# zubair-irshad/NeRF-MAE

Hardware: AMD Instinct MI355X
Metric: voxel-grids/sec (fwd+bwd+optimizer) swin_s 160^3 bf16 (higher is better)
Workload: dtype bf16; 1 GPU; swin_s MAE pretraining step, global batch 8 = 8 grid(s)/GPU of 4x160^3 RGB-sigma, mask_ratio 0.75, stochastic depth 0.1, AdamW+clip, DP=1 (BASELINE configs[2], the headline, read literally); global_batch=8, grids_per_gpu=8, resolution=160, parallelism=dp1, launch=hipgraph

## Files before the change

### nerf-mae_amd/csrc/common.hpp

```cpp
#pragma once
#include <hip/hip_runtime.h>
#include <stdint.h>

typedef unsigned short bf16_t;
typedef __attribute__((ext_vector_type(8))) short bf16x8;
typedef __attribute__((ext_vector_type(4))) short bf16x4;
typedef __attribute__((ext_vector_type(4))) float f32x4;
typedef __attribute__((ext_vector_type(4))) unsigned int u32x4;

#define NMH_DT_F32 0
#define NMH_DT_BF16 1

typedef float nmh_f2v __attribute__((ext_vector_type(2)));
typedef __bf16 nmh_b2v __attribute__((ext_vector_type(2)));
__device__ __forceinline__ unsigned pk_bf16(float lo, float hi) {
  nmh_f2v v = {lo, hi};
  return __builtin_bit_cast(unsigned, __builtin_convertvector(v, nmh_b2v));
}
__device__ __forceinline__ bf16_t f2bf(float f) { return __builtin_bit_cast(bf16_t, (__bf16)f); }
__device__ __forceinline__ float bf2f(bf16_t h) { return __uint_as_float(((unsigned)h) << 16); }

template <typename T> __device__ __forceinline__ float to_f(T v);
template <> __device__ __forceinline__ float to_f<float>(float v) { return v; }
template <> __device__ __forceinline__ float to_f<bf16_t>(bf16_t v) { return bf2f(v); }
// ... 71 lines not shown
  Frag<float> f;
  float4 a = *reinterpret_cast<const float4*>(lds + swz_off(row, 2 * g));
  float4 b = *reinterpret_cast<const float4*>(lds + swz_off(row, 2 * g + 1));
  f.v[0] = a.x; f.v[1] = a.y; f.v[2] = a.z; f.v[3] = a.w; f.v[4] = b.x; f.v[5] = b.y; f.v[6] = b.z; f.v[7] = b.w;
  return f;
}

typedef __attribute__((address_space(3))) bf16x4 lds_bf16x4;
__device__ __forceinline__ bf16x4 ds_read_tr16(const char* p) {
  return __builtin_amdgcn_ds_read_tr16_b64_v4i16((lds_bf16x4*)(__attribute__((address_space(3))) char*)p);
}
__device__ __forceinline__ Frag<bf16_t> lds_frag_t(const char* tile, int RS, int m0, int col0, int lane, bf16_t*) {
  const int g = lane >> 4, p = lane & 15;
  const char* a = tile + (m0 + 4 * g + (p >> 2)) * RS + (col0 + (p & 3) * 4) * 2;
  bf16x4 lo = ds_read_tr16(a);
  bf16x4 hi = ds_read_tr16(a + 16 * RS);
  Frag<bf16_t> f;
  f.v = __builtin_shufflevector(lo, hi, 0, 1, 2, 3, 4, 5, 6, 7);
  return f;
}
__device__ __forceinline__ Frag<float> lds_frag_t(const char* tile, int RS, int m0, int col0, int lane, float*) {
  const int g = lane >> 4, i = lane & 15;
  Frag<float> f;
#pragma unroll
  for (int j = 0; j < 8; ++j) {
    int m = m0 + 4 * g + (j & 3) + (j >> 2) * 16;
    f.v[j] = *reinterpret_cast<const float*>(tile + m * RS + (col0 + i) * 4);
  }
  return f;
}

struct TrFrag { bf16x4 lo, hi; };
__device__ __forceinline__ unsigned lds_addr_u(const void* p) { return (unsigned)(uintptr_t)(__attribute__((address_space(3))) const char*)p; }
template <int HI_OFF, int OFF0 = 0> __device__ __forceinline__ void tr_read_raw(TrFrag& f, unsigned addr) {
  static_assert(OFF0 >= 0 && OFF0 + HI_OFF < 65536, "ds offset field");
  asm volatile("ds_read_b64_tr_b16 %0, %1 offset:%2" : "=v"(f.lo) : "v"(addr), "n"(OFF0));
  asm volatile("ds_read_b64_tr_b16 %0, %1 offset:%2" : "=v"(f.hi) : "v"(addr), "n"(OFF0 + HI_OFF));
}
__device__ __forceinline__ float4 lds_read_f4_raw(const float* p) {
  float4 v;
  asm volatile("ds_read_b128 %0, %1\n\ts_waitcnt lgkmcnt(0)" : "=v"(v) : "v"(lds_addr_u(p)) : "memory");
  return v;
}
template <int OFF> __device__ __forceinline__ void tr_read1(bf16x4& d, unsigned addr) {
  static_assert(OFF >= 0 && OFF < 65536, "ds offset field");
  asm volatile("ds_read_b64_tr_b16 %0, %1 offset:%2" : "=v"(d) : "v"(addr), "n"(OFF));
}
__device__ __forceinline__ void tr_wait() { asm volatile("s_waitcnt lgkmcnt(0)" ::: "memory"); }
__device__ __forceinline__ void tr_pin(TrFrag& f) { asm volatile("" : "+v"(f.lo), "+v"(f.hi)); }
__device__ __forceinline__ Frag<bf16_t> tr_frag(const TrFrag& f) {
  Frag<bf16_t> r;
  r.v = __builtin_shufflevector(f.lo, f.hi, 0, 1, 2, 3, 4, 5, 6, 7);
  return r;
}

__device__ __forceinline__ float wave_sum(float v) {
#pragma unroll
  for (int o = 32; o > 0; o >>= 1) v += __shfl_xor(v, o, 64);
  return v;
}
__device__ __forceinline__ float gelu_f(float x) { return 0.5f * x * (1.0f + erff(x * 0.70710678118654752f)); }
__device__ __forceinline__ float gelu_grad_f(float x) {
  return 0.5f * (1.0f + erff(x * 0.70710678118654752f)) + x * 0.39894228040143268f * __expf(-0.5f * x * x);
}
__device__ __forceinline__ void erf_as_parts(float z, float& erfz, float& e) {
  const float az = fabsf(z);
  const float t = __builtin_amdgcn_rcpf(1.0f + 0.3275911f * az);
  e = __expf(-az * az);
  float p = 1.061405429f;
  p = p * t - 1.453152027f; p = p * t + 1.421413741f; p = p * t - 0.284496736f; p = p * t + 0.254829592f;
  erfz = copysignf(1.0f - p * t * e, z);
}
__device__ __forceinline__ float gelu_fast_f(float x) {
  float er, e;
  erf_as_parts(x * 0.70710678118654752f, er, e);
  return 0.5f * x * (1.0f + er);
}
__device__ __forceinline__ float gelu_grad_fast_f(float x) {
  float er, e;
  erf_as_parts(x * 0.70710678118654752f, er, e);
  return 0.5f * (1.0f + er) + x * 0.39894228040143268f * e;
}

struct NmhPerDeviceOnce {
  bool done[64] = {};
  static int dev() { int d = 0; if (hipGetDevice(&d) != hipSuccess || d < 0 || d >= 64) d = 0; return d; }
  bool need() const { return !done[dev()]; }
  void set() { done[dev()] = true; }
};
#ifdef __HIPCC__
static __global__ void nmh_zero_kernel(unsigned* p, long n) {
  for (long i = (long)blockIdx.x * blockDim.x + threadIdx.x; i < n; i += (long)gridDim.x * blockDim.x) p[i] = 0u;
}
extern char* g_nmh_arena_base;
extern size_t g_nmh_arena_bytes;
static inline hipError_t nmh_zero_async(void* p, size_t bytes, hipStream_t st) {
  const long n = (long)(bytes / 4);
  if (n <= 0) return hipSuccess;
  if (g_nmh_arena_bytes && (char*)p >= g_nmh_arena_base && (char*)p + bytes <= g_nmh_arena_base + g_nmh_arena_bytes) return hipSuccess;
  long nb = (n + 255) / 256;
  if (nb > 2048) nb = 2048;
  hipLaunchKernelGGL(nmh_zero_kernel, dim3((unsigned)nb), dim3(256), 0, st, (unsigned*)p, n);
  return hipGetLastError();
}
#endif
#define NMH_CHECK_LAUNCH() do { hipError_t e_ = hipGetLastError(); if (e_ != hipSuccess) return (int)e_; } while (0)
// ... 1 lines not shown
```

### nerf-mae_amd/csrc/conv48.hip

```cpp
#include "common.hpp"
#include "kernels.hpp"
#include <cstdlib>
#include <type_traits>

__device__ __forceinline__ unsigned c48_fdiv(unsigned n, const FDiv& f) { return f.sh < 0 ? n : (__umulhi(n, f.M) >> f.sh); }

namespace c48 {
constexpr int TZ = 4, TY = 8, TX = 16, HY = TY + 2, HX = TX + 2;
constexpr int LINE = HX * 96 + 16, PLANE = HY * LINE + 16, HALO = (TZ + 2) * PLANE;
constexpr int NSTEP = 41, CSTEPS = 9, WCHUNK = CSTEPS * 3 * 1024;
constexpr int LDS_BYTES = HALO + 2 * WCHUNK + 2 * 96 * 4;
constexpr int NLINE = (TZ + 2) * HY;
constexpr int LPW = (NLINE + 7) / 8;
constexpr int HREG = 2 * LPW;
static_assert(HREG == 16 && HX * 6 > 64 && HX * 6 <= 128, "the halo request schedule (4 per weight chunk 0-3) assumes 16 loads per thread, two per line");
static_assert(LINE % 32 == 16 && PLANE % 32 == 16, "bank-half alternation");
static_assert(LDS_BYTES <= 163840, "LDS budget");
}

struct C48Args {
  const bf16_t* X; const bf16_t* Wk; bf16_t* Y;
  int B, D, H, W, tz, ty, tx;
  long total;
  FDiv dtx, dty, dtz;
  int accumulate;
  double* stats_acc;
  const bf16_t* Y1; const float* stats1; float slope;
  float inv_slope;
  long wk_sample_stride;
  int ncib, ncob, ldx, ldy;
  int cosplit;
};

__device__ __forceinline__ void c48_tile_origin(const C48Args& a, long t, int& b, int& z0, int& y0, int& x0) {
  const unsigned tu = (unsigned)t;
  const unsigned r1 = c48_fdiv(tu, a.dtx), xt = tu - r1 * (unsigned)a.tx;
  const unsigned r2 = c48_fdiv(r1, a.dty), yt = r1 - r2 * (unsigned)a.ty;
  const unsigned r3 = c48_fdiv(r2, a.dtz), zt = r2 - r3 * (unsigned)a.tz;
  b = __builtin_amdgcn_readfirstlane((int)r3);
  z0 = __builtin_amdgcn_readfirstlane((int)zt * c48::TZ);
  y0 = __builtin_amdgcn_readfirstlane((int)yt * c48::TY);
  x0 = __builtin_amdgcn_readfirstlane((int)xt * c48::TX);
}

template <int, bool MB = false, bool RB = false, bool CZ = false>
__global__ __launch_bounds__(512) void conv48_kernel(C48Args a) {
  using namespace c48;
  constexpr long WBLK = (long)NSTEP * 3 * 512;
  extern __shared__ __attribute__((aligned(16))) char smem[];
  char* halo = smem;
  char* wbuf = smem + HALO;
  const int tid = threadIdx.x, lane = tid & 63, wave = tid >> 6, g = lane >> 4, li = lane & 15;

  const int nx = 8, xcd = blockIdx.x % nx, jb = blockIdx.x / nx, jstride = gridDim.x / nx;
  const bool split = MB && a.cosplit;
  const long total = split ? a.total * a.ncob : a.total;
  const long per = (total + nx - 1) / nx;
  const long tbeg = (long)xcd * per, tend = (tbeg + per < total) ? tbeg + per : total;

  uint4 hreg[HREG];
  const unsigned vox_bytes = MB ? (unsigned)a.ldx * 2u : 96u;
  const unsigned sample_bytes = (unsigned)a.D * a.H * a.W * vox_bytes;
  constexpr unsigned OOB = 0x80000000u;
  const int wv = __builtin_amdgcn_readfirstlane(wave);
  unsigned hv0 = OOB, hv1 = OOB;
  auto halo_voff = [&](int x0, int cib) {
    int lv = lane;
    asm volatile("" : "+v"(lv));
    const int c1 = lv + 64;
    const int hxa = (lv * 43) >> 8, hxb = (c1 * 43) >> 8;
    const int xa = x0 - 1 + hxa, xb = x0 - 1 + hxb;
    const unsigned cofs = MB ? (unsigned)cib * 96u : 0u;
    hv0 = (unsigned)xa < (unsigned)a.W ? (unsigned)xa * vox_bytes + (unsigned)(lv - hxa * 6) * 16u + cofs : OOB;
    hv1 = (c1 < HX * 6 && (unsigned)xb < (unsigned)a.W) ? (unsigned)xb * vox_bytes + (unsigned)(c1 - hxb * 6) * 16u + cofs : OOB;
  };
  auto halo_gload_one = [&](int i, int b, int z0, int y0, unsigned bytes) {
    const int j = i >> 1, l = wv + 8 * j;
    const int hz = (l * 205) >> 11, hy = l - hz * HY;
    const int z = z0 - 1 + hz, y = y0 - 1 + hy;
    const unsigned lok = (unsigned)(l < NLINE) & (unsigned)((unsigned)z < (unsigned)a.D) & (unsigned)((unsigned)y < (unsigned)a.H);
    const unsigned lmask = 0u - lok;
    const __amdgpu_buffer_rsrc_t rs = __builtin_amdgcn_make_buffer_rsrc((void*)(a.X + (long)b * (sample_bytes / 2)), 0, (int)(bytes & lmask), 0x00020000);
    const unsigned soff = ((unsigned)((z * a.H + y) * a.W) * vox_bytes) & lmask;
    hreg[i] = __builtin_bit_cast(uint4, __builtin_amdgcn_raw_buffer_load_b128(rs, (int)((i & 1) ? hv1 : hv0), (int)soff, 0));
  };
  auto halo_sstore = [&]() {
#pragma unroll
    for (int j = 0; j < LPW; ++j) {
      const int l = wv + 8 * j;
      if (l < NLINE) {
        const int hz = (l * 205) >> 11, hy = l - hz * HY;
        char* const p = halo + hz * PLANE + hy * LINE + lane * 16;
        *reinterpret_cast<uint4*>(p) = hreg[2 * j];
        if (lane < HX * 6 - 64) *reinterpret_cast<uint4*>(p + 1024) = hreg[2 * j + 1];
      }
    }
  };
  auto w_dma = [&](const bf16_t* wblk, int ck, int buf) {
    const int nunits = ((ck < 4) ? CSTEPS : (NSTEP - 4 * CSTEPS)) * 192;
    const char* src = reinterpret_cast<const char*>(wblk) + (long)ck * CSTEPS * 3072;
    char* dst = wbuf + buf * WCHUNK;
    for (int u0 = wave * 64; u0 < nunits; u0 += 512) {
      __builtin_amdgcn_global_load_lds((const __attribute__((address_space(1))) void*)(src + (long)(u0 + lane) * 16),
                                       (__attribute__((address_space(3))) void*)(dst + u0 * 16), 16, 0, 0);
    }
  };

  auto w_dma_one = [&](const bf16_t* wblk, int ck, int buf, int j) {
    const int nunits = ((ck < 4) ? CSTEPS : (NSTEP - 4 * CSTEPS)) * 192;
    const int u0 = wave * 64 + 512 * j;
    int lv = lane;
    asm volatile("" : "+v"(lv));
    if (u0 < nunits)
      __builtin_amdgcn_global_load_lds((const __attribute__((address_space(1))) void*)(reinterpret_cast<const char*>(wblk) + (long)ck * CSTEPS * 3072 + (long)(u0 + lv) * 16),
                                       (__attribute__((address_space(3))) void*)(wbuf + buf * WCHUNK + u0 * 16), 16, 0, 0);
  };

  for (int i = tid; i < HALO / 16; i += 512) reinterpret_cast<uint4*>(halo)[i] = make_uint4(0, 0, 0, 0);
  if (tid < 192) reinterpret_cast<float*>(smem + HALO + 2 * WCHUNK)[tid] = 0.f;
  __syncthreads();

  long t = tbeg + jb;
  if (t >= tend) return;
  int cb, cz0, cy0, cx0;
  c48_tile_origin(a, split ? t / a.ncob : t, cb, cz0, cy0, cx0);
  int cob = split ? (int)(t % a.ncob) : 0, cib = 0;
  const bf16_t* const wfirst = MB ? a.Wk + (long)cob * a.ncib * ((long)NSTEP * 3 * 512) : a.Wk + (long)cb * a.wk_sample_stride;
  halo_voff(cx0, 0);
#pragma unroll
  for (int i = 0; i < HREG; ++i) halo_gload_one(i, cb, cz0, cy0, sample_bytes);
  w_dma(wfirst, 0, 0);
  halo_sstore();
  __syncthreads();
  int wb = 0;

  const int z_l = wave >> 1, y_l = (wave & 1) * 4;
  const int base0 = z_l * PLANE + y_l * LINE + li * 96;
  int rowoff[2];
#pragma unroll
  for (int q = 0; q < 2; ++q) { const int r = 4 * q + g; rowoff[q] = (r / 3) * PLANE + (r % 3) * LINE; }
  const int row8 = 2 * PLANE + 2 * LINE;

  float* const sacc = reinterpret_cast<float*>(smem + HALO + 2 * WCHUNK);
  int st_b = -1, scur = 0;
  auto stats_flush = [&]() {
    if (st_b >= 0 && tid < 96) {
      float v = sacc[scur * 96 + tid];
      const float sacc_even = (RB && CZ) ? __shfl(v, (tid & 63) & ~1, 64) : 0.f;
      sacc[scur * 96 + tid] = 0.f;
      if (RB && (tid & 1)) {
        if constexpr (CZ) v -= a.stats1[(long)st_b * 96 + tid - 1] * sacc_even;
        v *= a.stats1[(long)st_b * 96 + tid];
      }
      atomicAdd(a.stats_acc + (long)st_b * 96 + tid, (double)v);
    }
  };
  auto row_sum = [](float v) -> float {
    v += __builtin_bit_cast(float, __builtin_amdgcn_update_dpp(0, __builtin_bit_cast(int, v), 0x111, 0xf, 0xf, true));
    v += __builtin_bit_cast(float, __builtin_amdgcn_update_dpp(0, __builtin_bit_cast(int, v), 0x112, 0xf, 0xf, true));
    v += __builtin_bit_cast(float, __builtin_amdgcn_update_dpp(0, __builtin_bit_cast(int, v), 0x114, 0xf, 0xf, true));
    v += __builtin_bit_cast(float, __builtin_amdgcn_update_dpp(0, __builtin_bit_cast(int, v), 0x118, 0xf, 0xf, true));
    return v;
  };
  f32x4 acc[4][3];
  for (;;) {
    long tn = t + jstride;
    int nco = 0, nci = 0;
    if (MB) {
      nci = cib + 1; nco = cob; tn = t;
      if (nci == a.ncib) { nci = 0; ++nco; }
      if (split) {
        if (nci == 0) { tn = t + jstride; nco = (int)(tn % a.ncob); }
      } else if (nco == a.ncob) { nco = 0; tn = t + jstride; }
    }
    const bool has_next = tn < tend;
    int nb = cb, nz0 = cz0, ny0 = cy0, nx0 = cx0;
    if (has_next && (!MB || tn != t)) c48_tile_origin(a, split ? tn / a.ncob : tn, nb, nz0, ny0, nx0);
    const unsigned nbytes = has_next ? sample_bytes : 0u;
    halo_voff(nx0, nci);
    const bf16_t* const wcur = MB ? a.Wk + (long)(cob * a.ncib + cib) * WBLK : a.Wk + (long)cb * a.wk_sample_stride;
    const bf16_t* const wnxt = MB ? a.Wk + (long)(nco * a.ncib + nci) * WBLK : a.Wk + (long)nb * a.wk_sample_stride;
    if (!MB || cib == 0) {
#pragma unroll
      for (int i = 0; i < 4; ++i)
#pragma unroll
        for (int n = 0; n < 3; ++n) acc[i][n] = f32x4{0.f, 0.f, 0.f, 0.f};
    }

    auto a_off = [&](int s) -> int {
      if (s < 36) {
        const int q = s / 18, c = s % 18;
        return base0 + rowoff[q] + (c / 6) * 96 + (c % 6) * 16;
      }
      int c = 4 * (s - 36) + g;
      c = c > 17 ? 17 : c;
      const int c6 = (c * 43) >> 8;
      return base0 + row8 + c6 * 96 + (c - 6 * c6) * 16;
    };
    Frag<bf16_t> bf[2][3], af[2][4];
    auto ld_frags = [&](int buf, const char* wsrc, int sl, int s) {
      const int ao = a_off(s);
#pragma unroll
      for (int n = 0; n < 3; ++n) bf[buf][n].v = *reinterpret_cast<const bf16x8*>(wsrc + (sl * 3 + n) * 1024 + lane * 16);
#pragma unroll
      for (int i = 0; i < 4; ++i) af[buf][i].v = *reinterpret_cast<const bf16x8*>(halo + ao + i * LINE);
    };
#pragma unroll
    for (int ck = 0; ck < 5; ++ck) {
      const int nxt = (ck < 4) ? ck + 1 : 0;
      const char* wsrc = wbuf + ((wb + ck) & 1) * WCHUNK;
      constexpr int NST4 = NSTEP - 4 * CSTEPS;
      const int nst = (ck < 4) ? CSTEPS : NST4;
      const int hbase = 4 * ck;
      const int hcnt = ck < 4 ? 4 : 0;
      ld_frags(0, wsrc, 0, ck * CSTEPS);
#pragma unroll
      for (int sl = 0; sl < CSTEPS; ++sl) {
        if (sl < nst) {
          if (sl + 1 < nst) ld_frags((sl + 1) & 1, wsrc, sl + 1, ck * CSTEPS + sl + 1);
          if (sl < 4) w_dma_one(ck < 4 ? wcur : wnxt, nxt, (wb + ck + 1) & 1, sl);
          if (sl >= 4) {
            const int k = (hcnt == 4) ? (sl == 4 ? 0 : sl == 5 ? 1 : sl == 6 ? 2 : sl == 8 ? 3 : -1) : (hcnt == 3) ? (sl == 4 ? 0 : sl == 6 ? 1 : sl == 8 ? 2 : -1) : -1;
            if (k >= 0) halo_gload_one(hbase + k, nb, nz0, ny0, nbytes);
          }
#pragma unroll
          for (int i = 0; i < 4; ++i)
#pragma unroll
            for (int n = 0; n < 3; ++n) mma(acc[i][n], bf[sl & 1][n], af[sl & 1][i]);
        }
      }
      if (hcnt == 4) asm volatile("s_waitcnt vmcnt(4)" ::: "memory");
      else if (hcnt == 3) asm volatile("s_waitcnt vmcnt(3)" ::: "memory");
      else asm volatile("s_waitcnt vmcnt(0)" ::: "memory");
      __builtin_amdgcn_s_barrier();
    }
    wb ^= 1;

    if (has_next) halo_sstore();

    if (!MB || cib == a.ncib - 1) {
      const int b = cb, z0 = cz0, y0 = cy0, x0 = cx0;
      const int z = z0 + z_l, x = x0 + li;
      const bool stats = !MB && a.stats_acc;
      if (stats && b != st_b) {
        stats_flush();
        if (st_b >= 0) scur ^= 1;
        st_b = b;
      }
      const int ldy = MB ? a.ldy : 48;
      bf16_t* const dst0 = a.Y + ((((long)b * a.D + z) * a.H + (y0 + y_l)) * a.W + x) * ldy + (MB ? cob * 48 : 0) + 12 * g;
      const long rowstride = (long)a.W * ldy;
      const bool zx_ok = z < a.D && x < a.W;
      auto epilogue = [&](auto with_stats) {
        constexpr bool ST = decltype(with_stats)::value;
        uint4 yA[RB ? 4 : 1]; uint2 yB[RB ? 4 : 1]; float4 mu4[RB ? 3 : 1];
        unsigned wk[RB ? 4 : 1][6];
        if constexpr (RB) {
          const bf16_t* const y1p = a.Y1 + (dst0 - a.Y);
#pragma unroll
          for (int i = 0; i < 4; ++i)
            if (zx_ok && y0 + y_l + i < a.H) {
              yA[i] = *reinterpret_cast<const uint4*>(y1p + i * rowstride);
              yB[i] = *reinterpret_cast<const uint2*>(y1p + i * rowstride + 8);
            }
          const float4* sp = reinterpret_cast<const float4*>(a.stats1 + ((long)b * 48 + 12 * g) * 2);
#pragma unroll
          for (int q = 0; q < 3; ++q) {
            const float4 p0 = sp[2 * q], p1 = sp[2 * q + 1];
            mu4[q] = make_float4(p0.x, p0.z, p1.x, p1.z);
          }
        }
        float st1[ST ? 3 : 1][4], st2[ST ? 3 : 1][4];
        if (ST) {
#pragma unroll
          for (int n = 0; n < 3; ++n)
#pragma unroll
            for (int r = 0; r < 4; ++r) { st1[ST ? n : 0][r] = 0.f; st2[ST ? n : 0][r] = 0.f; }
        }
#pragma unroll
        for (int i = 0; i < 4; ++i) {
          if (zx_ok && y0 + y_l + i < a.H) {
            bf16_t* dst = dst0 + i * rowstride;
            float v[3][4];
#pragma unroll
            for (int n = 0; n < 3; ++n)
#pragma unroll
              for (int r = 0; r < 4; ++r) v[n][r] = acc[i][n][r];
            if (a.accumulate) {
              const uint4 o = *reinterpret_cast<const uint4*>(dst);
              const uint2 o2 = *reinterpret_cast<const uint2*>(dst + 8);
              const unsigned ow[6] = {o.x, o.y, o.z, o.w, o2.x, o2.y};
// ... 9 lines not shown
#pragma unroll
              for (int q = 0; q < 6; ++q) wk[i][q] = w6[q];
            }
            if (ST && !RB) {
#pragma unroll
              for (int q = 0; q < 6; ++q) {
                const float q0 = __uint_as_float(w6[q] << 16), q1 = __uint_as_float(w6[q] & 0xffff0000u);
                st1[ST ? q >> 1 : 0][(q & 1) * 2] += q0; st1[ST ? q >> 1 : 0][(q & 1) * 2 + 1] += q1;
                st2[ST ? q >> 1 : 0][(q & 1) * 2] += q0 * q0; st2[ST ? q >> 1 : 0][(q & 1) * 2 + 1] += q1 * q1;
              }
            }
          }
        }
        if constexpr (RB) {
#pragma unroll
          for (int i = 0; i < 4; ++i)
            if (zx_ok && y0 + y_l + i < a.H) {
              const unsigned yw[6] = {yA[i].x, yA[i].y, yA[i].z, yA[i].w, yB[i].x, yB[i].y};
#pragma unroll
              for (int q = 0; q < 6; ++q) {
                const float d0 = __uint_as_float(wk[i][q] << 16), d1 = __uint_as_float(wk[i][q] & 0xffff0000u);
                const float m0 = (q & 1) ? mu4[q >> 1].z : mu4[q >> 1].x, m1 = (q & 1) ? mu4[q >> 1].w : mu4[q >> 1].y;
                const float y0v = __uint_as_float(yw[q] << 16), y1v = __uint_as_float(yw[q] & 0xffff0000u);
                if constexpr (CZ) {
                  const float g0 = d0 * (y0v > 0.f ? 1.0f : a.slope), g1 = d1 * (y1v > 0.f ? 1.0f : a.slope);
                  st1[q >> 1][(q & 1) * 2] += g0; st1[q >> 1][(q & 1) * 2 + 1] += g1;
                  st2[q >> 1][(q & 1) * 2] += d0 * y0v; st2[q >> 1][(q & 1) * 2 + 1] += d1 * y1v;
                } else {
                const float t0 = y0v - m0, t1 = y1v - m1;
                const float g0 = d0 * (t0 > 0.f ? 1.0f : a.slope), g1 = d1 * (t1 > 0.f ? 1.0f : a.slope);
                st1[q >> 1][(q & 1) * 2] += g0; st1[q >> 1][(q & 1) * 2 + 1] += g1;
                st2[q >> 1][(q & 1) * 2] += g0 * t0; st2[q >> 1][(q & 1) * 2 + 1] += g1 * t1;
                }
              }
            }
        }
        if (ST) {
#pragma unroll
          for (int n = 0; n < 3; ++n)
#pragma unroll
            for (int r = 0; r < 4; ++r) {
              const float a1 = row_sum(st1[ST ? n : 0][r]), a2 = row_sum(st2[ST ? n : 0][r]);
              if (li == 15) {
                float* dst = sacc + scur * 96 + (12 * g + 4 * n + r) * 2;
                atomicAdd(dst, a1);
                atomicAdd(dst + 1, a2);
              }
            }
        }
      };
      if (stats || RB) epilogue(std::true_type{});
      else epilogue(std::false_type{});
    }
    cb = nb; cz0 = nz0; cy0 = ny0; cx0 = nx0;
    __syncthreads();
    if (!has_next) break;
    t = tn; cob = nco; cib = nci;
  }
  if (a.stats_acc) stats_flush();
}


int k_conv48(const void* X, const void* Wk, void* Y, int B, int D, int H, int W, int accumulate, double* stats_acc, hipStream_t st,
             const void* Y1, const float* stats1, float slope, long wk_sample_stride, int centered) {
  using namespace c48;
  C48Args a;
  a.Y1 = (const bf16_t*)Y1; a.stats1 = stats1; a.slope = slope;
  a.inv_slope = slope != 0.f ? 1.0f / slope : 0.f; a.wk_sample_stride = wk_sample_stride;
  if (Y1 && (!stats1 || !stats_acc || accumulate)) return -1;
  if ((centered && !Y1) || (wk_sample_stride && (Y1 || accumulate))) return -1;
  a.X = (const bf16_t*)X; a.Wk = (const bf16_t*)Wk; a.Y = (bf16_t*)Y;
  a.B = B; a.D = D; a.H = H; a.W = W;
  a.tz = (D + TZ - 1) / TZ; a.ty = (H + TY - 1) / TY; a.tx = (W + TX - 1) / TX;
  a.total = (long)B * a.tz * a.ty * a.tx;
  if (a.total >= (1L << 31) || (long)D * H * W * 96 >= (1L << 31)) return -2;
  a.dtx = make_fdiv((unsigned)a.tx); a.dty = make_fdiv((unsigned)a.ty); a.dtz = make_fdiv((unsigned)a.tz);
  a.accumulate = accumulate;
  a.stats_acc = stats_acc;
  a.ncib = a.ncob = 1; a.ldx = a.ldy = 48; a.cosplit = 0;
  if (stats_acc) {
    hipError_t e = nmh_zero_async(stats_acc, sizeof(double) * 2 * 48 * B, st);
    if (e != hipSuccess) return (int)e;
  }
  static NmhPerDeviceOnce attr_set;
  if (attr_set.need()) {
    hipError_t e = hipFuncSetAttribute((const void*)conv48_kernel<0>, hipFuncAttributeMaxDynamicSharedMemorySize, LDS_BYTES);
    if (e != hipSuccess) return (int)e;
    attr_set.set();
  }
  long nb = a.total < 256 ? ((a.total + 7) / 8 * 8) : 256;
  if (Y1) {
    static NmhPerDeviceOnce attr_rb;
    if (attr_rb.need()) {
      hipError_t e = hipFuncSetAttribute((const void*)conv48_kernel<0, false, true>, hipFuncAttributeMaxDynamicSharedMemorySize, LDS_BYTES);
      if (e != hipSuccess) return (int)e;
      attr_rb.set();
    }
    if (centered) {
      static NmhPerDeviceOnce attr_cz;
      if (attr_cz.need()) {
        hipError_t e = hipFuncSetAttribute((const void*)conv48_kernel<0, false, true, true>, hipFuncAttributeMaxDynamicSharedMemorySize, LDS_BYTES);
        if (e != hipSuccess) return (int)e;
        attr_cz.set();
      }
      hipLaunchKernelGGL((conv48_kernel<0, false, true, true>), dim3((unsigned)nb), dim3(512), LDS_BYTES, st, a);
    } else hipLaunchKernelGGL((conv48_kernel<0, false, true>), dim3((unsigned)nb), dim3(512), LDS_BYTES, st, a);
    NMH_CHECK_LAUNCH();
    return 0;
  }
  hipLaunchKernelGGL(conv48_kernel<0>, dim3((unsigned)nb), dim3(512), LDS_BYTES, st, a);
  NMH_CHECK_LAUNCH();
  return 0;
// ... 258 lines not shown
    for (; bb < nblocks; ++bb) t8[bb & 7] += src[(long)bb * w48::PARTIAL];
    s = ((t8[0] * sc[0] + t8[1] * sc[1]) + (t8[2] * sc[2] + t8[3] * sc[3])) + ((t8[4] * sc[4] + t8[5] * sc[5]) + (t8[6] * sc[6] + t8[7] * sc[7]));
  }
  dW[((long)(os * 48 + ct * 16 + row) * Cin + cs * 48 + cit * 16 + col) * 27 + tap] += s;
}

long k_conv48_wgrad_ws_floats() { return 256L * w48::PARTIAL; }

static int launch_wgrad_halo(const void* dY, const void* X, float* dW, float* ws, int B, int D, int H, int W, int Cin, int Cout, hipStream_t st, const float* scale_stats = nullptr) {
  using namespace w48;
  W48Args a;
  a.X = (const bf16_t*)X; a.dY = (const bf16_t*)dY; a.ws = ws;
  a.B = B; a.D = D; a.H = H; a.W = W;
  a.tz = (D + TZ - 1) / TZ; a.ty = (H + TY - 1) / TY; a.tx = (W + TX - 1) / TX;
  a.total = (long)B * a.tz * a.ty * a.tx;
  if (a.total >= (1L << 31)) return -2;
  a.dtx = make_fdiv((unsigned)a.tx); a.dty = make_fdiv((unsigned)a.ty); a.dtz = make_fdiv((unsigned)a.tz);
  a.ldx = Cin; a.ldy = Cout; a.nci = Cin / 48;
  const int nsub = (Cin / 48) * (Cout / 48);
  static NmhPerDeviceOnce attr_set;
  if (attr_set.need()) {
    hipError_t e = hipFuncSetAttribute((const void*)conv48_wgrad_kernel, hipFuncAttributeMaxDynamicSharedMemorySize, LDS_BYTES);
    if (e != hipSuccess) return (int)e;
    attr_set.set();
  }
  if (scale_stats) {
    const long tps = (long)a.tz * a.ty * a.tx;
    if (nsub != 1 || B < 1 || 8 % B || tps % (8 / B)) return -2;
  }
  int nb;
  if (nsub == 1) nb = a.total < 256 ? (int)((a.total + 7) / 8 * 8) : 256;
  else {
    static const int side_wgs = [] { const char* e = getenv("NMH_W48_SIDE_WGS"); const int v = e ? atoi(e) : 128; return v < 1 ? 1 : (v > 256 ? 256 : v); }();
    nb = side_wgs / nsub;
    if (nb < 1) nb = 1;
    if (nb > a.total) nb = (int)a.total;
  }
  hipLaunchKernelGGL(conv48_wgrad_kernel, dim3(nb, nsub), dim3(512), LDS_BYTES, st, a);
  NMH_CHECK_LAUNCH();
  hipLaunchKernelGGL(conv48_wgrad_reduce_kernel, dim3((PARTIAL + 255) / 256, nsub), dim3(256), 0, st, ws, dW, nb, a.nci, Cin, scale_stats, B);
  NMH_CHECK_LAUNCH();
  return 0;
}
int k_conv48_wgrad(const void* dY, const void* X, float* dW, float* ws, int B, int D, int H, int W, hipStream_t st, const float* scale_stats) {
  return launch_wgrad_halo(dY, X, dW, ws, B, D, H, W, 48, 48, st, scale_stats);
}

__global__ void conv48_pack_scaled_kernel(const float* __restrict__ W, const float* __restrict__ stats, bf16_t* __restrict__ out) {
  constexpr int IMG = c48::NSTEP * 3 * 512;
  const int b = blockIdx.y;
  for (int iw = blockIdx.x * 256 + threadIdx.x; iw < IMG; iw += gridDim.x * 256) {
    const int j = iw & 7, lane = (iw >> 3) & 63, sn = iw >> 9;
    const int nt = sn % 3, st = sn / 3, g = lane >> 4, li = lane & 15, n = 12 * (li >> 2) + 4 * nt + (li & 3);
    int r, c;
    if (st < 36) { r = 4 * (st / 18) + g; c = st % 18; } else { r = 8; c = 4 * (st - 36) + g; }
    float v = 0.f;
    if (c < 18) {
      const int tap = r * 3 + c / 6, k = (c % 6) * 8 + j;
      v = W[((long)n * 48 + k) * 27 + tap] * stats[((long)b * 48 + k) * 2 + 1];
    }
    out[(long)b * IMG + iw] = f2bf(v);
  }
}
int k_conv48_pack_scaled(const float* W, const float* stats, void* out, int B, hipStream_t st) {
  hipLaunchKernelGGL(conv48_pack_scaled_kernel, dim3(62, B), dim3(256), 0, st, W, stats, (bf16_t*)out);
  NMH_CHECK_LAUNCH();
  return 0;
}
int k_conv3_wgrad_halo(const void* dY, const void* X, float* dW, float* ws, int B, int D, int H, int W, int Cin, int Cout, hipStream_t st) {
  if (Cin % 48 || Cout % 48 || (Cin / 48) * (Cout / 48) > 256 || (double)D * H * W * Cin * 2 >= 4294967296.0) return -2;
  return launch_wgrad_halo(dY, X, dW, ws, B, D, H, W, Cin, Cout, st);
}
```

### nerf-mae_amd/csrc/misc.hip

```cpp
#include "common.hpp"
#include "kernels.hpp"

static inline unsigned ew_blocks(long total, int cap = 16384) { long nb = (total + 255) / 256; return (unsigned)(nb > cap ? cap : (nb < 1 ? 1 : nb)); }

template <typename T> __global__ __launch_bounds__(256) void embed_gather_kernel(const float* __restrict__ x, T* __restrict__ A, int B, int R) {
  extern __shared__ __attribute__((aligned(16))) char esm[];
  const int g = R >> 2;
  constexpr int ROWB = 256 * (int)sizeof(T) + 8;
  const int line = blockIdx.x;
  const int ty = line % g, tz = (line / g) % g, b = line / (g * g);
  for (int idx = threadIdx.x; idx < 64 * g; idx += 256) {
    const int q = idx / g, tx = idx - q * g;
    const int ci = q >> 4, kz = (q >> 2) & 3, ky = q & 3;
    const float4 v = *reinterpret_cast<const float4*>(x + ((((long)b * 4 + ci) * R + 4 * tz + kz) * R + 4 * ty + ky) * (long)R + 4 * tx);
    T* o = reinterpret_cast<T*>(esm + tx * ROWB) + q * 4;
    o[0] = from_f<T>(v.x); o[1] = from_f<T>(v.y); o[2] = from_f<T>(v.z); o[3] = from_f<T>(v.w);
  }
  __syncthreads();
  constexpr int V8 = 256 * (int)sizeof(T) / 8;
  unsigned long long* out = reinterpret_cast<unsigned long long*>(A + (long)line * g * 256);
  for (int idx = threadIdx.x; idx < g * V8; idx += 256) {
    const int tx = idx / V8, c = idx - tx * V8;
    out[idx] = *reinterpret_cast<const unsigned long long*>(esm + tx * ROWB + c * 8);
  }
// ... 456 lines not shown
  p.g = tokmask ? g : 0;
  hipLaunchKernelGGL(step_params_kernel, dim3(n ? (n + 255) / 256 : 1), dim3(256), 0, st, p, tokmask, hyper_dev, ext_dev);
  NMH_CHECK_LAUNCH();
  return 0;
}

__global__ void grad_f32_to_bf16_kernel(const float* __restrict__ src, bf16_t* __restrict__ dst, long n8) {
  for (long i = (long)blockIdx.x * blockDim.x + threadIdx.x; i < n8; i += (long)gridDim.x * blockDim.x) {
    float v[8];
    Vec8<float>::load(src + i * 8, v);
    Vec8<bf16_t>::store(dst + i * 8, v);
  }
}
__global__ void grad_bf16_to_f32_kernel(const bf16_t* __restrict__ src, float* __restrict__ dst, long n8, float scale) {
  for (long i = (long)blockIdx.x * blockDim.x + threadIdx.x; i < n8; i += (long)gridDim.x * blockDim.x) {
    float v[8];
    Vec8<bf16_t>::load(src + i * 8, v);
#pragma unroll
    for (int j = 0; j < 8; ++j) v[j] *= scale;
    Vec8<float>::store(dst + i * 8, v);
  }
}
int k_grad_cast(int to_bf16, const void* src, void* dst, long n, float scale, hipStream_t st) {
  if (n % 8 || ((uintptr_t)src | (uintptr_t)dst) & 15) return -2;
  if (to_bf16) hipLaunchKernelGGL(grad_f32_to_bf16_kernel, dim3(ew_blocks(n / 8)), dim3(256), 0, st, (const float*)src, (bf16_t*)dst, n / 8);
  else hipLaunchKernelGGL(grad_bf16_to_f32_kernel, dim3(ew_blocks(n / 8)), dim3(256), 0, st, (const bf16_t*)src, (float*)dst, n / 8, scale);
  NMH_CHECK_LAUNCH();
  return 0;
}
__global__ void fill_kernel(float* p, float v, long n) {
  for (long i = (long)blockIdx.x * blockDim.x + threadIdx.x; i < n; i += (long)gridDim.x * blockDim.x) p[i] = v;
}
int k_fill_f32(float* p, float v, long n, hipStream_t st) {
  hipLaunchKernelGGL(fill_kernel, dim3(ew_blocks(n)), dim3(256), 0, st, p, v, n);
  NMH_CHECK_LAUNCH();
  return 0;
}

__device__ __forceinline__ long pack_src_index(const PackDesc& d, long il) {
  const unsigned i = (unsigned)il, d0 = (unsigned)d.d0, d1 = (unsigned)d.d1, d2 = (unsigned)d.d2;
  switch (d.mode) {
    case 1: { unsigned c = i / d0, r = i - c * d0; return (long)(r * d1 + c); }
    case 2: { unsigned t2 = i / d1, ci = i - t2 * d1, co = t2 / 27u, t = t2 - co * 27u; return (long)((co * d1 + ci) * 27u + t); }
    case 3: { unsigned t2 = i / d0, co = i - t2 * d0, ci = t2 / 27u, t = t2 - ci * 27u; return (long)((co * d1 + ci) * 27u + (26u - t)); }
    case 4: { unsigned t2 = i / d0, ci = i - t2 * d0, t = t2 / d1, co = t2 - t * d1; return (long)((ci * d1 + co) * d2 + t); }
    case 5: { unsigned n = d1 * d2, ci = i / n, r = i - ci * n, t = r / d1, co = r - t * d1; return (long)((ci * d1 + co) * d2 + t); }
    case 6: case 7: {
      constexpr unsigned IMG = 41u * 3u * 512u;
      const unsigned blk = i / IMG, iw = i - blk * IMG;
      const unsigned nkb = (d.mode == 6 ? d1 : d0) / 48u, ob = blk / nkb, kb = blk - ob * nkb;
      const int j = (int)(iw & 7), lane = (int)((iw >> 3) & 63);
      const unsigned sn = iw >> 9;
      const int nt = (int)(sn % 3), st = (int)(sn / 3), g = lane >> 4, li = lane & 15, n = (int)ob * 48 + 12 * (li >> 2) + 4 * nt + (li & 3);
      int r, c;
      if (st < 36) { r = 4 * (st / 18) + g; c = st % 18; } else { r = 8; c = 4 * (st - 36) + g; }
      if (c >= 18) return -1;
      const int tap = r * 3 + c / 6, k = (int)kb * 48 + (c % 6) * 8 + j;
      return d.mode == 6 ? ((long)n * d1 + k) * 27 + tap : ((long)k * d1 + n) * 27 + (26 - tap);
    }
    case 10: { unsigned r = i / d1; return r < d0 ? (long)i : -1; }
    case 11: { unsigned c = i / d2, r = i - c * d2; return r < d0 ? (long)(r * d1 + c) : -1; }
    case 12: { unsigned ci = i & 7u, t2 = i >> 3, co = t2 / d2, t = t2 - co * d2; return ci < d1 ? (long)((co * d1 + ci) * d2 + t) : -1; }
    case 8: case 9: {
      const int j = (int)(i & 7), lane = (int)((i >> 3) & 63);
      const unsigned sn = i >> 9;
      const int nt = (int)(sn & 3), sg = (int)(sn >> 2), blk = sg / 54, st = sg - blk * 54;
      const int ncs = (d.mode == 8 ? (int)d1 : (int)d0) / 64, os = blk / ncs, cs = blk - os * ncs;
      const int g = lane >> 4, li = lane & 15, n = os * 64 + 16 * (li >> 2) + 4 * nt + (li & 3), k = cs * 64 + (st & 1) * 32 + 8 * g + j, tap = st >> 1;
      return d.mode == 8 ? ((long)n * d1 + k) * 27 + tap : ((long)k * d1 + n) * 27 + (26 - tap);
    }
    default: return il;
  }
}
template <typename T> __global__ void pack_kernel(const PackDesc* descs, const int* blk2desc, const long* blkstart) {
  const PackDesc d = descs[blk2desc[blockIdx.x]];
  const long base = blkstart[blockIdx.x];
  T* dst = (T*)d.dst;
  if (d.mode == 1) {
    __shared__ float tile[32][33];
    const int tcn = (d.d1 + 31) >> 5, tr = (int)(base / tcn), tc = (int)(base - (long)tr * tcn);
    const int r0 = tr * 32, c0 = tc * 32, tx = threadIdx.x & 31, ty = threadIdx.x >> 5;
#pragma unroll
    for (int r = ty; r < 32; r += 8)
      if (r0 + r < d.d0 && c0 + tx < d.d1) tile[r][tx] = d.src[(long)(r0 + r) * d.d1 + c0 + tx];
    __syncthreads();
#pragma unroll
    for (int c = ty; c < 32; c += 8)
      if (c0 + c < d.d1 && r0 + tx < d.d0) dst[(long)(c0 + c) * d.d0 + r0 + tx] = from_f<T>(tile[tx][c]);
    return;
  }
  if (d.mode == 2 || d.mode == 3) {
    __shared__ float tl[32][28];
    const int Co = d.d0, Ci = d.d1, tx = threadIdx.x & 31, ty = threadIdx.x >> 5;
    if (d.mode == 2) {
      const int cchunks = (Ci + 31) >> 5, co = (int)(base / cchunks), ci0 = (int)(base - (long)co * cchunks) * 32;
      const float* sp = d.src + ((long)co * Ci + ci0) * 27;
      const int nci = Ci - ci0 < 32 ? Ci - ci0 : 32;
      for (int i = threadIdx.x; i < nci * 27; i += 256) tl[i / 27][i % 27] = sp[i];
      __syncthreads();
      for (int t = ty; t < 27; t += 8)
        if (tx < nci) dst[((long)co * 27 + t) * Ci + ci0 + tx] = from_f<T>(tl[tx][t]);
    } else {
      const int ochunks = (Co + 31) >> 5, ci = (int)(base / ochunks), co0 = (int)(base - (long)ci * ochunks) * 32;
      const int nco = Co - co0 < 32 ? Co - co0 : 32;
      for (int i = threadIdx.x; i < nco * 27; i += 256) { const int c = i / 27, t = i - c * 27; tl[c][t] = d.src[((long)(co0 + c) * Ci + ci) * 27 + t]; }
      __syncthreads();
      for (int t = ty; t < 27; t += 8)
        if (tx < nco) dst[((long)ci * 27 + t) * Co + co0 + tx] = from_f<T>(tl[tx][26 - t]);
    }
    return;
// ... 269 lines not shown
```

Before: 193.9 grids/s.

## Stream conv48 halo via buffer_load-to-LDS DMA in two channel halves

```diff
diff --git a/nerf-mae_amd/csrc/common.hpp b/nerf-mae_amd/csrc/common.hpp
--- a/nerf-mae_amd/csrc/common.hpp
+++ b/nerf-mae_amd/csrc/common.hpp
@@ -147,6 +147,20 @@
   Frag<bf16_t> r;
   r.v = __builtin_shufflevector(f.lo, f.hi, 0, 1, 2, 3, 4, 5, 6, 7);
   return r;
+}
+
+__host__ __device__ inline bool c48_slot(int st, int g, int& h, int& r, int& c) {
+  const int s2 = st >= 21 ? st - 21 : st;
+  if (s2 < 18) {
+    h = st >= 21;
+    r = s2 < 9 ? g + ((g + 1) >> 1) : (g < 2 ? 6 + 2 * g : 3 * g - 5);
+    c = s2 < 9 ? s2 : s2 - 9;
+    return true;
+  }
+  r = 7;
+  if (st <= 20) { const int u = 4 * (st - 18) + g; h = u > 8; c = h ? u - 9 : u; return true; }
+  h = 1; c = 3 + 4 * (st - 39) + g;
+  return c < 9;
 }
 
 __device__ __forceinline__ float wave_sum(float v) {
diff --git a/nerf-mae_amd/csrc/conv48.hip b/nerf-mae_amd/csrc/conv48.hip
--- a/nerf-mae_amd/csrc/conv48.hip
+++ b/nerf-mae_amd/csrc/conv48.hip
@@ -7,14 +7,14 @@
 
 namespace c48 {
 constexpr int TZ = 4, TY = 8, TX = 16, HY = TY + 2, HX = TX + 2;
-constexpr int LINE = HX * 96 + 16, PLANE = HY * LINE + 16, HALO = (TZ + 2) * PLANE;
+constexpr int VOX = 48, LCH = HX * 3;
+constexpr int LINE = HX * VOX + 32, PLANE = HY * LINE, HALF = (TZ + 2) * PLANE, HALO = 2 * HALF;
 constexpr int NSTEP = 41, CSTEPS = 9, WCHUNK = CSTEPS * 3 * 1024;
 constexpr int LDS_BYTES = HALO + 2 * WCHUNK + 2 * 96 * 4;
 constexpr int NLINE = (TZ + 2) * HY;
 constexpr int LPW = (NLINE + 7) / 8;
-constexpr int HREG = 2 * LPW;
-static_assert(HREG == 16 && HX * 6 > 64 && HX * 6 <= 128, "the halo request schedule (4 per weight chunk 0-3) assumes 16 loads per thread, two per line");
-static_assert(LINE % 32 == 16 && PLANE % 32 == 16, "bank-half alternation");
+static_assert(LPW == 8 && LCH <= 64 && LPW <= CSTEPS, "one DMA instruction per line, one line per k-step of a 9-step weight chunk");
+static_assert(LINE % 256 == 128 && PLANE % 256 == 0 && HALF % 256 == 0, "tap rows paired in a ds_read_b128 service group are a multiple of 256 B apart");
 static_assert(LDS_BYTES <= 163840, "LDS budget");
 }
 
@@ -43,6 +43,23 @@
   x0 = __builtin_amdgcn_readfirstlane((int)xt * c48::TX);
 }
 
+__device__ __forceinline__ void c48_halo_dma(u32x4 rsrc, unsigned voff, unsigned soff, unsigned lds_dst, unsigned long long lanes) {
+  unsigned keep_m0;
+  unsigned long long keep_exec;
+  asm volatile(
+      "s_mov_b32 %0, m0\n\t"
+      "s_mov_b64 %1, exec\n\t"
+      "s_mov_b32 m0, %5\n\t"
+      "s_mov_b64 exec, %6\n\t"
+      "s_nop 0\n\t"
+      "buffer_load_dwordx4 %2, %3, %4 offen lds\n\t"
+      "s_mov_b64 exec, %1\n\t"
+      "s_mov_b32 m0, %0"
+      : "=&s"(keep_m0), "=&s"(keep_exec)
+      : "v"(voff), "s"(rsrc), "s"(soff), "s"(lds_dst), "s"(lanes)
+      : "memory");
+}
+
 template <int, bool MB = false, bool RB = false, bool CZ = false>
 __global__ __launch_bounds__(512) void conv48_kernel(C48Args a) {
   using namespace c48;
@@ -58,43 +75,30 @@
   const long per = (total + nx - 1) / nx;
   const long tbeg = (long)xcd * per, tend = (tbeg + per < total) ? tbeg + per : total;
 
-  uint4 hreg[HREG];
   const unsigned vox_bytes = MB ? (unsigned)a.ldx * 2u : 96u;
   const unsigned sample_bytes = (unsigned)a.D * a.H * a.W * vox_bytes;
   constexpr unsigned OOB = 0x80000000u;
   const int wv = __builtin_amdgcn_readfirstlane(wave);
-  unsigned hv0 = OOB, hv1 = OOB;
-  auto halo_voff = [&](int x0, int cib) {
+  const unsigned halo_u = lds_addr_u(halo);
+  auto halo_voff = [&](int x0, int cib) -> unsigned {
     int lv = lane;
     asm volatile("" : "+v"(lv));
-    const int c1 = lv + 64;
-    const int hxa = (lv * 43) >> 8, hxb = (c1 * 43) >> 8;
-    const int xa = x0 - 1 + hxa, xb = x0 - 1 + hxb;
+    const int hx = (lv * 43) >> 7;
+    const int x = x0 - 1 + hx;
     const unsigned cofs = MB ? (unsigned)cib * 96u : 0u;
-    hv0 = (unsigned)xa < (unsigned)a.W ? (unsigned)xa * vox_bytes + (unsigned)(lv - hxa * 6) * 16u + cofs : OOB;
-    hv1 = (c1 < HX * 6 && (unsigned)xb < (unsigned)a.W) ? (unsigned)xb * vox_bytes + (unsigned)(c1 - hxb * 6) * 16u + cofs : OOB;
-  };
-  auto halo_gload_one = [&](int i, int b, int z0, int y0, unsigned bytes) {
-    const int j = i >> 1, l = wv + 8 * j;
+    return (unsigned)x < (unsigned)a.W ? (unsigned)x * vox_bytes + (unsigned)(lv - hx * 3) * 16u + cofs : OOB;
+  };
+  auto halo_dma_one = [&](int j, int half, int b, int z0, int y0, unsigned voff, bool on) {
+    const int l = wv + 8 * j;
     const int hz = (l * 205) >> 11, hy = l - hz * HY;
     const int z = z0 - 1 + hz, y = y0 - 1 + hy;
-    const unsigned lok = (unsigned)(l < NLINE) & (unsigned)((unsigned)z < (unsigned)a.D) & (unsigned)((unsigned)y < (unsigned)a.H);
+    const unsigned lok = (unsigned)((unsigned)z < (unsigned)a.D) & (unsigned)((unsigned)y < (unsigned)a.H);
     const unsigned lmask = 0u - lok;
-    const __amdgpu_buffer_rsrc_t rs = __builtin_amdgcn_make_buffer_rsrc((void*)(a.X + (long)b * (sample_bytes / 2)), 0, (int)(bytes & lmask), 0x00020000);
-    const unsigned soff = ((unsigned)((z * a.H + y) * a.W) * vox_bytes) & lmask;
-    hreg[i] = __builtin_bit_cast(uint4, __builtin_amdgcn_raw_buffer_load_b128(rs, (int)((i & 1) ? hv1 : hv0), (int)soff, 0));
-  };
-  auto halo_sstore = [&]() {
-#pragma unroll
-    for (int j = 0; j < LPW; ++j) {
-      const int l = wv + 8 * j;
-      if (l < NLINE) {
-        const int hz = (l * 205) >> 11, hy = l - hz * HY;
-        char* const p = halo + hz * PLANE + hy * LINE + lane * 16;
-        *reinterpret_cast<uint4*>(p) = hreg[2 * j];
-        if (lane < HX * 6 - 64) *reinterpret_cast<uint4*>(p + 1024) = hreg[2 * j + 1];
-      }
-    }
+    const unsigned long long xb = (unsigned long long)(a.X + (long)b * (sample_bytes / 2));
+    const u32x4 rs = {(unsigned)xb, (unsigned)(xb >> 32) & 0xffffu, sample_bytes & lmask, 0x00020000u};
+    const unsigned soff = (((unsigned)((z * a.H + y) * a.W) * vox_bytes) & lmask) + (unsigned)half * VOX;
+    const unsigned long long em = ((unsigned)(l < NLINE) & (unsigned)on) ? (1ull << LCH) - 1 : 0ull;
+    c48_halo_dma(rs, voff, soff, halo_u + (unsigned)(half * HALF + hz * PLANE + hy * LINE), em);
   };
   auto w_dma = [&](const bf16_t* wblk, int ck, int buf) {
     const int nunits = ((ck < 4) ? CSTEPS : (NSTEP - 4 * CSTEPS)) * 192;
@@ -116,7 +120,6 @@
                                        (__attribute__((address_space(3))) void*)(wbuf + buf * WCHUNK + u0 * 16), 16, 0, 0);
   };
 
-  for (int i = tid; i < HALO / 16; i += 512) reinterpret_cast<uint4*>(halo)[i] = make_uint4(0, 0, 0, 0);
   if (tid < 192) reinterpret_cast<float*>(smem + HALO + 2 * WCHUNK)[tid] = 0.f;
   __syncthreads();
 
@@ -126,20 +129,20 @@
   c48_tile_origin(a, split ? t / a.ncob : t, cb, cz0, cy0, cx0);
   int cob = split ? (int)(t % a.ncob) : 0, cib = 0;
   const bf16_t* const wfirst = MB ? a.Wk + (long)cob * a.ncib * ((long)NSTEP * 3 * 512) : a.Wk + (long)cb * a.wk_sample_stride;
-  halo_voff(cx0, 0);
-#pragma unroll
-  for (int i = 0; i < HREG; ++i) halo_gload_one(i, cb, cz0, cy0, sample_bytes);
+  unsigned hvc = halo_voff(cx0, 0);
+#pragma unroll
+  for (int j = 0; j < LPW; ++j) halo_dma_one(j, 0, cb, cz0, cy0, hvc, true);
   w_dma(wfirst, 0, 0);
-  halo_sstore();
+  asm volatile("s_waitcnt vmcnt(0)" ::: "memory");
   __syncthreads();
   int wb = 0;
 
   const int z_l = wave >> 1, y_l = (wave & 1) * 4;
-  const int base0 = z_l * PLANE + y_l * LINE + li * 96;
+  const int base0 = z_l * PLANE + y_l * LINE + li * VOX;
   int rowoff[2];
 #pragma unroll
-  for (int q = 0; q < 2; ++q) { const int r = 4 * q + g; rowoff[q] = (r / 3) * PLANE + (r % 3) * LINE; }
-  const int row8 = 2 * PLANE + 2 * LINE;
+  for (int q = 0; q < 2; ++q) { int h, r, c; c48_slot(9 * q, g, h, r, c); rowoff[q] = (r / 3) * PLANE + (r % 3) * LINE; }
+  const int row7 = 2 * PLANE + 1 * LINE;
 
   float* const sacc = reinterpret_cast<float*>(smem + HALO + 2 * WCHUNK);
   int st_b = -1, scur = 0;
@@ -176,8 +179,7 @@
     const bool has_next = tn < tend;
     int nb = cb, nz0 = cz0, ny0 = cy0, nx0 = cx0;
     if (has_next && (!MB || tn != t)) c48_tile_origin(a, split ? tn / a.ncob : tn, nb, nz0, ny0, nx0);
-    const unsigned nbytes = has_next ? sample_bytes : 0u;
-    halo_voff(nx0, nci);
+    const unsigned hvn = halo_voff(nx0, nci);
     const bf16_t* const wcur = MB ? a.Wk + (long)(cob * a.ncib + cib) * WBLK : a.Wk + (long)cb * a.wk_sample_stride;
     const bf16_t* const wnxt = MB ? a.Wk + (long)(nco * a.ncib + nci) * WBLK : a.Wk + (long)nb * a.wk_sample_stride;
     if (!MB || cib == 0) {
@@ -188,14 +190,13 @@
     }
 
     auto a_off = [&](int s) -> int {
-      if (s < 36) {
-        const int q = s / 18, c = s % 18;
-        return base0 + rowoff[q] + (c / 6) * 96 + (c % 6) * 16;
-      }
-      int c = 4 * (s - 36) + g;
-      c = c > 17 ? 17 : c;
-      const int c6 = (c * 43) >> 8;
-      return base0 + row8 + c6 * 96 + (c - 6 * c6) * 16;
+      if (s < 18) return base0 + rowoff[s / 9] + (s % 9) * 16;
+      if (s >= 21 && s < 39) return base0 + HALF + rowoff[(s - 21) / 9] + ((s - 21) % 9) * 16;
+      if (s < 20) return base0 + row7 + (4 * (s - 18) + g) * 16;
+      if (s == 20) return base0 + row7 + (g == 0 ? 8 * 16 : HALF + (g - 1) * 16);
+      int c = 3 + 4 * (s - 39) + g;
+      c = c > 8 ? 8 : c;
+      return base0 + HALF + row7 + c * 16;
     };
     Frag<bf16_t> bf[2][3], af[2][4];
     auto ld_frags = [&](int buf, const char* wsrc, int sl, int s) {
@@ -211,32 +212,28 @@
       const char* wsrc = wbuf + ((wb + ck) & 1) * WCHUNK;
       constexpr int NST4 = NSTEP - 4 * CSTEPS;
       const int nst = (ck < 4) ? CSTEPS : NST4;
-      const int hbase = 4 * ck;
-      const int hcnt = ck < 4 ? 4 : 0;
       ld_frags(0, wsrc, 0, ck * CSTEPS);
 #pragma unroll
       for (int sl = 0; sl < CSTEPS; ++sl) {
         if (sl < nst) {
           if (sl + 1 < nst) ld_frags((sl + 1) & 1, wsrc, sl + 1, ck * CSTEPS + sl + 1);
+          if (sl < LPW) {
+            if (ck == 0) halo_dma_one(sl, 1, cb, cz0, cy0, hvc, true);
+            if (ck == 3) halo_dma_one(sl, 0, nb, nz0, ny0, hvn, has_next);
+          }
           if (sl < 4) w_dma_one(ck < 4 ? wcur : wnxt, nxt, (wb + ck + 1) & 1, sl);
-          if (sl >= 4) {
-            const int k = (hcnt == 4) ? (sl == 4 ? 0 : sl == 5 ? 1 : sl == 6 ? 2 : sl == 8 ? 3 : -1) : (hcnt == 3) ? (sl == 4 ? 0 : sl == 6 ? 1 : sl == 8 ? 2 : -1) : -1;
-            if (k >= 0) halo_gload_one(hbase + k, nb, nz0, ny0, nbytes);
-          }
 #pragma unroll
           for (int i = 0; i < 4; ++i)
 #pragma unroll
             for (int n = 0; n < 3; ++n) mma(acc[i][n], bf[sl & 1][n], af[sl & 1][i]);
         }
       }
-      if (hcnt == 4) asm volatile("s_waitcnt vmcnt(4)" ::: "memory");
-      else if (hcnt == 3) asm volatile("s_waitcnt vmcnt(3)" ::: "memory");
+      if (ck == 0 || ck == 3) asm volatile("s_waitcnt vmcnt(4)" ::: "memory");
       else asm volatile("s_waitcnt vmcnt(0)" ::: "memory");
       __builtin_amdgcn_s_barrier();
     }
     wb ^= 1;
 
-    if (has_next) halo_sstore();
 
     if (!MB || cib == a.ncib - 1) {
       const int b = cb, z0 = cz0, y0 = cy0, x0 = cx0;
@@ -352,12 +349,14 @@
       if (stats || RB) epilogue(std::true_type{});
       else epilogue(std::false_type{});
     }
-    cb = nb; cz0 = nz0; cy0 = ny0; cx0 = nx0;
-    __syncthreads();
+    cb = nb; cz0 = nz0; cy0 = ny0; cx0 = nx0; hvc = hvn;
     if (!has_next) break;
     t = tn; cob = nco; cib = nci;
   }
-  if (a.stats_acc) stats_flush();
+  if (a.stats_acc) {
+    __syncthreads();
+    stats_flush();
+  }
 }
 
 
@@ -722,11 +721,10 @@
   for (int iw = blockIdx.x * 256 + threadIdx.x; iw < IMG; iw += gridDim.x * 256) {
     const int j = iw & 7, lane = (iw >> 3) & 63, sn = iw >> 9;
     const int nt = sn % 3, st = sn / 3, g = lane >> 4, li = lane & 15, n = 12 * (li >> 2) + 4 * nt + (li & 3);
-    int r, c;
-    if (st < 36) { r = 4 * (st / 18) + g; c = st % 18; } else { r = 8; c = 4 * (st - 36) + g; }
+    int h, r, c;
     float v = 0.f;
-    if (c < 18) {
-      const int tap = r * 3 + c / 6, k = (c % 6) * 8 + j;
+    if (c48_slot(st, g, h, r, c)) {
+      const int tap = r * 3 + c / 3, k = h * 24 + (c % 3) * 8 + j;
       v = W[((long)n * 48 + k) * 27 + tap] * stats[((long)b * 48 + k) * 2 + 1];
     }
     out[(long)b * IMG + iw] = f2bf(v);
diff --git a/nerf-mae_amd/csrc/misc.hip b/nerf-mae_amd/csrc/misc.hip
--- a/nerf-mae_amd/csrc/misc.hip
+++ b/nerf-mae_amd/csrc/misc.hip
@@ -532,10 +532,9 @@
       const int j = (int)(iw & 7), lane = (int)((iw >> 3) & 63);
       const unsigned sn = iw >> 9;
       const int nt = (int)(sn % 3), st = (int)(sn / 3), g = lane >> 4, li = lane & 15, n = (int)ob * 48 + 12 * (li >> 2) + 4 * nt + (li & 3);
-      int r, c;
-      if (st < 36) { r = 4 * (st / 18) + g; c = st % 18; } else { r = 8; c = 4 * (st - 36) + g; }
-      if (c >= 18) return -1;
-      const int tap = r * 3 + c / 6, k = (int)kb * 48 + (c % 6) * 8 + j;
+      int h, r, c;
+      if (!c48_slot(st, g, h, r, c)) return -1;
+      const int tap = r * 3 + c / 3, k = (int)kb * 48 + h * 24 + (c % 3) * 8 + j;
       return d.mode == 6 ? ((long)n * d1 + k) * 27 + tap : ((long)k * d1 + n) * 27 + (26 - tap);
     }
     case 10: { unsigned r = i / d1; return r < d0 ? (long)i : -1; }
```

Result: no change. 195.1 grids/s, median of 6 (+0.6%).
